# zovoilis-lab/Flye

Measured on AMD Instinct MI355X. Metric: Gbp reads overlapped/sec, higher is better.
Workload: dtype u64

## Files before the change

flye_amd/csrc/fg_ctx.h:

```cpp
#pragma once

#include <hip/hip_runtime.h>
#include <cstdint>
#include <cstdio>
#include <cstdlib>
#include <new>
#include <cstring>
#include <string>
#include <vector>
#include <map>
#include <memory>
#include <condition_variable>
#include <functional>
#include <mutex>
#include <thread>
#include <atomic>
#include <algorithm>

#include "../../include/flye_gpu.h"
#include "fg_error.h"

typedef uint64_t u64;
typedef uint32_t u32;
typedef uint16_t u16;
// ... 252 lines not shown
	std::vector<i32> hQLen;
	DevBuf<u64> dQWords, dQWordOff;
	DevBuf<i32> dQLen;

	bool indexBuilt = false;
	float sampleRate = 1.0f;
	u64 nKeys = 0, nEntries = 0, nRep = 0, tableSlots = 0;
	DevBuf<u64> dKeys;
	DevBuf<u64> dKeyOff;
	DevBuf<u64> dEntries;
	DevBuf<u64> dRepKeys;
	DevBuf<u64> dTable;
	bool tableWide = false;
	FgTable table{};
	DevBuf<u32> dIndexedBits;
	DevBuf<u32> dMaybeBits;
	u32 shardWorld = 1, shardRank = 0;

	std::unique_ptr<fg_ctx> lane2;
	std::shared_ptr<void> indexBuild;
	bool gathering = false;
	DevBuf<u64> gKeys, gKeyOff, gEntries, gRepKeys;
	u64 gNKeys = 0, gNEntries = 0, gNRep = 0;
	u32 splitWorld = 0;
	DevBuf<u64> sCounts, sEntries;
	bool scattering = false;
	u32 scatterWorld = 1, scatterRank = 0;

	DevBuf<u32> dQuery;
	u64 hitCapHint = 0;
	const u32* curQuery = nullptr;
	DevBuf<u64> dQKmerOff;
	DevBuf<u64> dProbe;
	DevBuf<u64> dPartK0, dPartV0, dPartK1, dPartV1;
	DevBuf<char> dPartScratch;
	DevBuf<unsigned long long> dPartCount;
	DevBuf<u64> dHitOff;
	DevBuf<u64> dFiltOff;
	DevBuf<i32> dFiltPos;
	DevBuf<u64> dHitKey;
	DevBuf<u32> dHitVal;
	DevBuf<u16> dHitVal16;
	bool hitVal16 = false;
	DevBuf<u32> dHitKey32;
	DevBuf<i32> dScore, dBack;
	DevBuf<int4> dCand;
	DevBuf<u64> dGroupStart;
	DevBuf<u32> dGroupQuery;
	DevBuf<u32> dGroupExt, dGroupFirstCur, dGroupLastCur;
	DevBuf<uint8_t> dGroupExtSorted;
	DevBuf<u32> dTmp32;
	DevBuf<fg_seed_hit> dSeedHits;
	DevBuf<u64> dRecvRun, dRecvIdx;
	DevBuf<u32> dRecvErr;
	DevBuf<u64> dCntA, dCntB, dGroupCnt, dGroupOff, dPrimCnt, dPrimOff, dDpGroups, dDpElems;
	DevBuf<u32> dPrimFlag, dDpSize, dListSmall, dListBig, dListDp, dListFused, dListCnt;
	DevBuf<u32> dTileCnt, dPrimPos, dScanScratch;
	DevBuf<u32> dCur, dExt;
	DevBuf<char> dPrimOut;
	DevBuf<u64> dPrimNode, dPrimBase, dMatchSize, dMatchOff, dMatches;
	DevBuf<u32> dMatchCnt;
	PinnedBuf<u64> hMatches, hMatchOff;
	PinnedBuf<u32> hMatchCnt;
	DevBuf<char> dSortTasks, dSortBig;
	DevBuf<unsigned long long> dSmallElems;
	DevBuf<unsigned long long> dLazyCnt;
// ... 385 lines not shown
```

flye_amd/csrc/fg_overlap.hip:

```cpp
#include "fg_ctx.h"
#include "fg_wavesort.h"
#include "fg_devprim.h"
#include "fg_taskchain.h"
#include <atomic>

#include <algorithm>
#include <cmath>
#include <chrono>
#include <functional>
#include <thread>
#include <type_traits>

#define WG 256
#define FLAG_SELF (1ULL << 63)
#define FLAG_FLIP (1ULL << 62)
#define OFF_MASK ((1ULL << 38) - 1)

namespace {

__device__ __forceinline__ u32 block_exscan(u32 v, u32* sh , u32* total)
{
	const int lane = threadIdx.x & 63, w = threadIdx.x >> 6;
	u32 inc = v;
	for (int o = 1; o < 64; o <<= 1)
// ... 281 lines not shown
				const u64 own = ((u64)(rec ^ (fl ? 1u : 0u)) << 32) | (u32)(fl ? L - pq - k : pq);
				if (pe >= own) pe = e;
				if (e >= own) e = entries[(so & OFF_MASK) + j + 1];
			}
			if (tieFree)
			{
				const u32 below = (u32)__builtin_amdgcn_update_dpp((int)(u32)(pe >> 32), (int)(u32)(e >> 32), 0x138, 0xf, 0xf, false);
				tied |= j > 0 && below == (u32)(e >> 32);
			}
			u32 srec = (u32)(e >> 32);
			i32 spos = (i32)(u32)e;
			if (so & FLAG_FLIP) { spos = len[srec >> 1] - spos - k; srec ^= 1u; }
			if constexpr (std::is_same<KT, fg_seed_hit>::value)
				hitKey[hbase + o] = fg_seed_hit{p0 + (i32)t, spos, firstId + srec};
			else if constexpr (std::is_same<KT, PK>::value)
				hitKey[hbase + o] = PK(((u64)srec << (curBits + FG_PK_VALBITS)) | ((u64)(u32)(p0 + (i32)t) << FG_PK_VALBITS) |
									   (u64)(u32)spos);
			else
			{
				if (sizeof(KT) == 8) hitKey[hbase + o] = (KT)(((u64)(firstId + srec) << 32) | (u32)(p0 + (i32)t));
				else hitKey[hbase + o] = (KT)((srec << curBits) | (u32)(p0 + (i32)t));
				hitVal[hbase + o] = (VT)(u32)spos;
			}
		}
		__syncthreads();
		hbase += tot;
		fbase += ftot;
	}
	if (tieFree)
	{
		const int anyTied = __syncthreads_or(tied);
		if (threadIdx.x == 0) tieFree[q] = anyTied ? 0u : 1u;
	}
}


__global__ void k_filt_pos(const u64* __restrict__ qKmerOff, const u64* __restrict__ probe, const u64* __restrict__ filtOff,
						   i32* __restrict__ filtPos)
{
	__shared__ u32 sh[WG / 64 + 1];
	const u32 q = blockIdx.x;
	const u64 a = qKmerOff[q];
	const i32 nk = (i32)(qKmerOff[q + 1] - a);
	u64 fbase = filtOff[q];
	for (i32 p0 = 0; p0 < nk; p0 += WG)
	{
		const i32 p = p0 + (i32)threadIdx.x;
		const u64 v = p < nk ? probe[a + p] : 0;
		const u32 rep = (v != 0 && (u32)(v & FG_CNT_MASK) == FG_CNT_REPETITIVE) ? 1u : 0u;
		u32 tot;
		const u32 off = block_exscan(rep, sh, &tot);
		if (rep) filtPos[fbase + off] = p;
		fbase += tot;
	}
}

__global__ void k_recv_keys(const u32* __restrict__ query, const u64* __restrict__ qKmerOff, const u64* __restrict__ qWords,
							const u64* __restrict__ qWordOff, const i32* __restrict__ qLen, const i32* __restrict__ len, int k,
							u32 firstId, u32 nRec, const fg_seed_hit* __restrict__ hits, const u64* __restrict__ run, u32 nSrc,
							const u64* __restrict__ hitOff, int recBits, int posBits, int mode, u64* __restrict__ keys,
							u64* __restrict__ vals, u64* __restrict__ hitIdx, u32* __restrict__ err)
{
	const u32 q = blockIdx.x;
	const u32 rec = query[q];
	const i32 nk = qLen[rec >> 1] - k;
	const bool rc = rec & 1;
// ... 1311 lines not shown
		const u64 n = localOff[q1] - localOff[q0];
		if (n)
		{
			c->dPartK0.reserve(n); c->dPartV0.reserve(n); c->dPartK1.reserve(n); c->dPartV1.reserve(n);
			c->dPartScratch.reserve(fgprim::radixSortScratchBytes(n));
			c->dPartCount.reserve(1);
			HIP_CHECK(hipMemsetAsync(c->dPartCount.p, 0, 8, s));
			{ ScopedK t(c->timer, "k_probe_emit");
			  hipLaunchKernelGGL(k_probe_emit, q1 - q0, WG, 0, s, q0, c->dQuery.p, qWords, qWordOff, qLen, c->dKmerOff.p, c->dQKmerOff.p,
								 c->k, c->table, regionShift, c->hasQ ? (const u32*)nullptr : c->dIndexedBits.p, probeSkipBits(c),
								 n, c->dPartK0.p, c->dPartV0.p, c->dPartCount.p); }
			unsigned long long nEmit = 0;
			HIP_CHECK(hipMemcpyAsync(&nEmit, c->dPartCount.p, 8, hipMemcpyDeviceToHost, s));
			HIP_CHECK(hipStreamSynchronize(s));
			if (nEmit > n) throw FgError{FG_ERR_HIP, "internal: more probe pairs than query k-mers"};
			if (nEmit == 0) { q0 = q1; continue; }
			int which;
			{ ScopedK t(c->timer, "k_probe_partition");
			  which = fgprim::radixSortPairs(s, c->dPartK0.p, c->dPartV0.p, c->dPartK1.p, c->dPartV1.p, nEmit, PART_KEY_BITS,
											 PART_KEY_BITS + PROBE_REGION_BITS, c->dPartScratch.p); }
			{ ScopedK t(c->timer, "k_probe");
			  hipLaunchKernelGGL(k_probe_sorted, (unsigned)((nEmit + WG - 1) / WG), WG, 0, s, which ? c->dPartK1.p : c->dPartK0.p,
								 which ? c->dPartV1.p : c->dPartV0.p, (u64)nEmit, c->table, c->dProbe.p,
								 getenv("FG_ABLATE_PROBE") ? atoi(getenv("FG_ABLATE_PROBE")) : 0); }
		}
		q0 = q1;
	}
	{ ScopedK t(c->timer, "k_probe_count");
	  hipLaunchKernelGGL(k_probe_count, nq, WG, 0, s, c->dQKmerOff.p, c->dProbe.p, c->dCntA.p, c->dCntB.p); }
}

struct ChunkResult { u64 nPrim, nHits, dpGroups, dpElems, dpElemsSmall, nMatchSlots; };

static void probeChunk(fg_ctx* c, const u32* hq, const u64* hQKmerOff, u32 qa, u32 qb, std::vector<u64>& hitsPerQuery)
{
	hipStream_t s = c->stream;
	const int k = c->k;
	const u32 nq = qb - qa;
	const u64 totalQK = hQKmerOff[qb] - hQKmerOff[qa];
	std::vector<u64> localOff(nq + 1);
	for (u32 i = 0; i <= nq; ++i) localOff[i] = hQKmerOff[qa + i] - hQKmerOff[qa];
	c->dQuery.reserve(nq); c->dQKmerOff.reserve(nq + 1);
	c->dProbe.reserve(totalQK);
	c->dHitOff.reserve(nq + 1); c->dFiltOff.reserve(nq + 1);
	c->dCntA.reserve(nq + 1); c->dCntB.reserve(nq + 1); c->dGroupCnt.reserve(nq + 1); c->dGroupOff.reserve(nq + 1);
	c->dPrimCnt.reserve(nq + 1); c->dPrimOff.reserve(nq + 1); c->dDpGroups.reserve(nq + 1); c->dDpElems.reserve(nq + 1);
	c->dListCnt.reserve(4);
	HIP_CHECK(hipMemcpyAsync(c->dQuery.p, hq + qa, nq * 4ULL, hipMemcpyHostToDevice, s));
	HIP_CHECK(hipMemcpyAsync(c->dQKmerOff.p, localOff.data(), (nq + 1) * 8ULL, hipMemcpyHostToDevice, s));

	const u64* qWords = c->hasQ ? c->dQWords.p : c->dWords.p;
	const u64* qWordOff = c->hasQ ? c->dQWordOff.p : c->dWordOff.p;
	const i32* qLen = c->hasQ ? c->dQLen.p : c->dLen.p;
	const bool partition = !c->tableWide && c->k <= 17 &&
		(getenv("FG_PROBE_PARTITION") ? atoi(getenv("FG_PROBE_PARTITION")) != 0 : false);
	if (partition) probePartitioned(c, nq, localOff.data(), qWords, qWordOff, qLen);
	else
	{ ScopedK t(c->timer, "k_probe");
	  const u32* skipBits = probeSkipBits(c);
	  if (c->tableWide)
		hipLaunchKernelGGL(k_probe<true>, nq, WG, 0, s, c->dQuery.p, qWords, qWordOff, qLen, c->dKmerOff.p,
						   c->dQKmerOff.p, k, c->table, c->hasQ ? (const u32*)nullptr : c->dIndexedBits.p, skipBits,
						   c->dProbe.p, c->dCntA.p, c->dCntB.p);
	  else
		hipLaunchKernelGGL(k_probe<false>, nq, WG, 0, s, c->dQuery.p, qWords, qWordOff, qLen, c->dKmerOff.p,
						   c->dQKmerOff.p, k, c->table, c->hasQ ? (const u32*)nullptr : c->dIndexedBits.p, skipBits,
						   c->dProbe.p, c->dCntA.p, c->dCntB.p); }
	hitsPerQuery.resize(nq);
	HIP_CHECK(hipMemcpyAsync(hitsPerQuery.data(), c->dCntA.p, nq * 8ULL, hipMemcpyDeviceToHost, s));
	HIP_CHECK(hipStreamSynchronize(s));
}

template <class KT>
static void recvFill(fg_ctx* c, const RecvHits* recv, u32 callQ0, u32 sub0, u32 nq, u64 nHits, int curBits, KT* hitKey, u32* hitVal)
{
	hipStream_t s = c->stream;
	const int k = c->k;
	const u32* dQuery = c->dQuery.p + sub0;
	const u64* dQKmerOff = c->dQKmerOff.p + sub0;
	{ ScopedK t(c->timer, "k_filt_pos");
	  hipLaunchKernelGGL(k_filt_pos, nq, WG, 0, s, dQKmerOff, c->dProbe.p, c->dFiltOff.p, c->dFiltPos.p); }
	if (nHits == 0) return;
	if (nHits > fgprim::RS_MAX_N) throw FgError{FG_ERR_ARG, "more than 2^30 - 1 seed hits in one sub-range"};
	const u32 ns = recv->nSrc;
	std::vector<u64> run(2 * (size_t)nq * ns);
	for (u32 i = 0; i < nq; ++i)
		for (u32 src = 0; src < ns; ++src)
		{
			const size_t at = (size_t)(callQ0 + sub0 + i) * ns + src;
// ... 24 lines not shown
						 c->dHitOff.p, recBits, posBits, onePass ? 0 : 1, c->dPartK0.p, c->dPartV0.p, c->dRecvIdx.p, c->dRecvErr.p); }
	if (fetchScalar(c, c->dRecvErr.p)) throw FgError{FG_ERR_ARG, "a received seed hit lies outside its query or its target"};
	u64 *k0 = c->dPartK0.p, *v0 = c->dPartV0.p, *k1 = c->dPartK1.p, *v1 = c->dPartV1.p;
	{ ScopedK t(c->timer, "k_recv_sort");
	  if (fgprim::radixSortPairs(s, k0, v0, k1, v1, nHits, 0, onePass ? gBits + storedBits : storedBits, c->dPartScratch.p))
		  { std::swap(k0, k1); std::swap(v0, v1); } }
	if (!onePass)
	{
		{ ScopedK t(c->timer, "k_recv_keys");
		  hipLaunchKernelGGL(k_recv_gkey, (unsigned)((nHits + WG - 1) / WG), WG, 0, s, v0, nHits, c->dHitOff.p, nq, dQKmerOff,
							 recv->hits, c->dRecvIdx.p, k0); }
		ScopedK t(c->timer, "k_recv_sort");
		if (fgprim::radixSortPairs(s, k0, v0, k1, v1, nHits, 0, gBits, c->dPartScratch.p)) { std::swap(k0, k1); std::swap(v0, v1); }
	}
	{ ScopedK t(c->timer, "k_recv_place");
	  hipLaunchKernelGGL(k_recv_place<KT>, (unsigned)((nHits + WG - 1) / WG), WG, 0, s, v0, nHits, recv->hits, c->dRecvIdx.p,
						 c->firstId, curBits, hitKey, hitVal); }
}

static void deviceSub(fg_ctx* c, const fg_detector_params* p, uint8_t forceLocal, u32 sub0, u32 nq, u64 primBase,
					  u64 hitCapHint , ChunkResult* res,
					  const RecvHits* recv = nullptr, u32 callQ0 = 0)
{
	hipStream_t s = c->stream;
	const int k = c->k;
	const u32* dQuery = c->dQuery.p + sub0;
	const u64* dQKmerOff = c->dQKmerOff.p + sub0;
	c->curQuery = dQuery;
	const i32* qLen = c->hasQ ? c->dQLen.p : c->dLen.p;
	c->dHitOff.reserve(nq + 1); c->dFiltOff.reserve(nq + 1);
	c->dGroupCnt.reserve(nq + 1); c->dGroupOff.reserve(nq + 1);
	c->dPrimCnt.reserve(nq + 1); c->dPrimOff.reserve(nq + 1); c->dDpGroups.reserve(nq + 1); c->dDpElems.reserve(nq + 1);
	c->dListCnt.reserve(4);
	{ ScopedK t(c->timer, "k_exscan");
	  hipLaunchKernelGGL(k_exscan, 1, 1024, 0, s, c->dCntA.p + sub0, c->dHitOff.p, nq);
	  hipLaunchKernelGGL(k_exscan, 1, 1024, 0, s, c->dCntB.p + sub0, c->dFiltOff.p, nq); }
	c->hScalar.reserve(8);
	HIP_CHECK(hipMemcpyAsync(c->hScalar.p, c->dHitOff.p + nq, 8, hipMemcpyDeviceToHost, s));
	HIP_CHECK(hipMemcpyAsync(c->hScalar.p + 1, c->dFiltOff.p + nq, 8, hipMemcpyDeviceToHost, s));
	HIP_CHECK(hipStreamSynchronize(s));
	const u64 nHits = c->hScalar.p[0], nFilt = c->hScalar.p[1];
	res->nHits = nHits;
	const u64 hitCap = std::max(nHits, hitCapHint);
	c->hitCapHint = hitCap;
	c->dFiltPos.reserve(nFilt + 1);
	int curBits = 1, recBits = 1;
	while ((1LL << curBits) < (long long)(c->hasQ ? c->qMaxLen : c->maxLen)) ++curBits;
	while ((1ULL << recBits) < 2ULL * c->nReads) ++recBits;
	const bool key32 = curBits + recBits <= 32 && !getenv("FG_FORCE_KEY64");
	c->tieFreeN = 0; c->sortReasonN = 0;
	const bool canPack = recBits + curBits + FG_PK_VALBITS <= 64 && c->maxLen < (1 << FG_PK_VALBITS);
	const bool wantPack = !(getenv("FG_PACKED_KEYS") && atoi(getenv("FG_PACKED_KEYS")) == 0);
	const int keyMode = key32 ? 0 : ((canPack && wantPack) ? 1 : 2);
	const bool val16 = keyMode == 0 && !recv && c->maxLen <= 65536 && !(getenv("FG_VAL16") && atoi(getenv("FG_VAL16")) == 0);
	c->hitVal16 = val16;
	if (keyMode == 0)
	{
		c->dHitKey32.reserve(hitCap + 1); c->dTieFree.reserve(nq + 1);
		if (val16) c->dHitVal16.reserve(hitCap + 2); else c->dHitVal.reserve(hitCap + 1);
		if (recv) recvFill<u32>(c, recv, callQ0, sub0, nq, nHits, curBits, c->dHitKey32.p, c->dHitVal.p);
		else { ScopedK t(c->timer, "k_fill");
		  if (val16)
			  hipLaunchKernelGGL((k_fill<u32, u16>), nq, WG, 0, s, dQuery, c->dLen.p, qLen, dQKmerOff, k, c->firstId, curBits,
								 c->dProbe.p, c->dEntries.p, c->dHitOff.p, c->dFiltOff.p, c->dHitKey32.p, c->dHitVal16.p, c->dFiltPos.p, c->dTieFree.p);
		  else
			  hipLaunchKernelGGL(k_fill<u32>, nq, WG, 0, s, dQuery, c->dLen.p, qLen, dQKmerOff, k, c->firstId, curBits,
								 c->dProbe.p, c->dEntries.p, c->dHitOff.p, c->dFiltOff.p, c->dHitKey32.p, c->dHitVal.p, c->dFiltPos.p, c->dTieFree.p); }
		if (!recv) { c->tieFreeQ0 = callQ0 + sub0; c->tieFreeN = nq; }
		const u32* sortFree = recv ? nullptr : c->dTieFree.p;
		if (sortFree && nHits)
		{
			c->dSortFree.reserve(nq + 1); c->dSortReason.reserve(nq + 1);
			if (sortScreen(c, c->dHitOff.p, nq, c->dHitKey32.p, curBits, recBits, c->dTieFree.p, fgChainMinUnique(p), p->min_overlap,
						   c->dSortFree.p, c->dSortReason.p))
				{ sortFree = c->dSortFree.p; c->sortReasonN = nq; }
		}
		if (val16) sortSegments<u32, u16>(c, c->dHitOff.p, nq, c->dHitKey32.p, c->dHitVal16.p, nHits, curBits, sortFree, recBits);
		else sortSegments<u32>(c, c->dHitOff.p, nq, c->dHitKey32.p, c->dHitVal.p, nHits, curBits, sortFree, recBits);
	}
	else if (keyMode == 1)
	{
		c->dHitKey.reserve(hitCap + 1);
		if (recv) recvFill<PK>(c, recv, callQ0, sub0, nq, nHits, curBits, (PK*)c->dHitKey.p, (u32*)nullptr);
		else { ScopedK t(c->timer, "k_fill");
		  hipLaunchKernelGGL(k_fill<PK>, nq, WG, 0, s, dQuery, c->dLen.p, qLen, dQKmerOff, k, c->firstId, curBits,
							 c->dProbe.p, c->dEntries.p, c->dHitOff.p, c->dFiltOff.p, (PK*)c->dHitKey.p, (u32*)nullptr, c->dFiltPos.p, (u32*)nullptr); }
		sortSegments<PK>(c, c->dHitOff.p, nq, (PK*)c->dHitKey.p, (u32*)nullptr, nHits, curBits);
	}
	else
	{
		c->dHitKey.reserve(hitCap + 1); c->dHitVal.reserve(hitCap + 1);
		if (recv) recvFill<u64>(c, recv, callQ0, sub0, nq, nHits, curBits, c->dHitKey.p, c->dHitVal.p);
		else { ScopedK t(c->timer, "k_fill");
		  hipLaunchKernelGGL(k_fill<u64>, nq, WG, 0, s, dQuery, c->dLen.p, qLen, dQKmerOff, k, c->firstId, 0,
							 c->dProbe.p, c->dEntries.p, c->dHitOff.p, c->dFiltOff.p, c->dHitKey.p, c->dHitVal.p, c->dFiltPos.p, (u32*)nullptr); }
		sortSegments<u64>(c, c->dHitOff.p, nq, c->dHitKey.p, c->dHitVal.p, nHits, curBits);
	}
	const HitKeyView<u32> hk32{c->dHitKey32.p, c->dHitVal.p, curBits, c->firstId};
	const HitKeyView<u64> hk64{c->dHitKey.p, c->dHitVal.p, curBits, c->firstId};
	const HitKeyView<PK> hkp{(const PK*)c->dHitKey.p, nullptr, curBits, c->firstId};
	const bool flat = nHits < 0xFFFFFFFFULL && !(getenv("FG_GROUP_FLAT") && atoi(getenv("FG_GROUP_FLAT")) == 0);
	const u64 nTiles = (nHits + FG_GROUP_TILE - 1) / FG_GROUP_TILE;
	u64 nGroups = 0;
	if (!flat)
	{
		{ ScopedK t(c->timer, "k_group_count");
		  if (keyMode == 0) hipLaunchKernelGGL(k_group_count<u32>, nq, WG, 0, s, c->dHitOff.p, hk32, c->dGroupCnt.p);
		  else if (keyMode == 1) hipLaunchKernelGGL(k_group_count<PK>, nq, WG, 0, s, c->dHitOff.p, hkp, c->dGroupCnt.p);
		  else hipLaunchKernelGGL(k_group_count<u64>, nq, WG, 0, s, c->dHitOff.p, hk64, c->dGroupCnt.p); }
		{ ScopedK t(c->timer, "k_exscan");
		  hipLaunchKernelGGL(k_exscan, 1, 1024, 0, s, c->dGroupCnt.p, c->dGroupOff.p, nq); }
		nGroups = fetchScalar(c, c->dGroupOff.p + nq);
	}
	else if (nTiles)
	{
		c->dTileCnt.reserve(nTiles + 1); c->dScanScratch.reserve(fgprim::scanScratchElems(nTiles + 1));
		{ ScopedK t(c->timer, "k_group_count");
		  if (keyMode == 0) hipLaunchKernelGGL((k_group_count_flat<u32, FG_GROUP_GF>), (unsigned)nTiles, WG, 0, s, c->dHitOff.p, nq, hk32, nHits, c->dTileCnt.p);
		  else if (keyMode == 1) hipLaunchKernelGGL((k_group_count_flat<PK, FG_GROUP_GF>), (unsigned)nTiles, WG, 0, s, c->dHitOff.p, nq, hkp, nHits, c->dTileCnt.p);
		  else hipLaunchKernelGGL((k_group_count_flat<u64, FG_GROUP_GF>), (unsigned)nTiles, WG, 0, s, c->dHitOff.p, nq, hk64, nHits, c->dTileCnt.p); }
		{ ScopedK t(c->timer, "k_group_scan");
		  fgprim::scan<u32>(s, c->dTileCnt.p, c->dTileCnt.p, nTiles + 1, false, c->dScanScratch.p); }
		nGroups = fetchScalar(c, c->dTileCnt.p + nTiles);
	}
	if (nGroups >= 0xFFFFFFFFULL) throw FgError{FG_ERR_ARG, "too many target groups in one chunk"};
// ... 106 lines not shown
	  }
	  HIP_CHECK(hipMemcpyAsync(c->hOff.p + 3 * (size_t)(nq + 1), c->dSmallElems.p, 24, hipMemcpyDeviceToHost, s));
	  HIP_CHECK(hipEventRecord(c->evOff, s));
	  static const int wantPieces = getenv("FG_D2H_PIECES") ? std::max(1, std::min(FG_D2H_MAX_PIECES, atoi(getenv("FG_D2H_PIECES")))) : 12;
	  const int nPieces = nPrim >= 100000 ? wantPieces : 1;
	  for (int i = 0; i < nPieces; ++i)
	  {
		  const u64 a = nPrim * i / nPieces, b = nPrim * (i + 1) / nPieces;
		  if (b > a)
			  HIP_CHECK(hipMemcpyAsync(c->hPrim.p + (primBase + a) * sizeof(PrimRec), c->dPrimOut.p + a * sizeof(PrimRec),
									   (b - a) * sizeof(PrimRec), hipMemcpyDeviceToHost, s));
		  HIP_CHECK(hipEventRecord(c->evPiece[i], s));
		  c->pieceEnd[i] = primBase + b;
	  }
	  c->nPieces = nPieces; }
	HIP_CHECK(hipEventSynchronize(c->evOff));
	if (keepAln) HIP_CHECK(hipStreamSynchronize(s));
	res->nPrim = nPrim;
	res->dpGroups = 0; res->dpElems = 0;
	res->dpElemsSmall = c->hOff.p[3 * (size_t)(nq + 1)];
	if (flat) { res->dpGroups = c->hOff.p[3 * (size_t)(nq + 1) + 1]; res->dpElems = c->hOff.p[3 * (size_t)(nq + 1) + 2]; }
	else for (u32 i = 0; i < nq; ++i) { res->dpGroups += c->hOff.p[(nq + 1) + i]; res->dpElems += c->hOff.p[2 * (size_t)(nq + 1) + i]; }
}

static void stageBudgets(fg_ctx* c, u64& kmerBudget, u64& hitBudget)
{
	kmerBudget = getenv("FG_KMER_BUDGET") ? strtoull(getenv("FG_KMER_BUDGET"), nullptr, 10) : (1ULL << 30);
	hitBudget = getenv("FG_HIT_BUDGET") ? strtoull(getenv("FG_HIT_BUDGET"), nullptr, 10) : (3ULL << 29);
	if (!getenv("FG_KMER_BUDGET") && !getenv("FG_HIT_BUDGET"))
	{
		size_t freeB = 0, totalB = 0;
		HIP_CHECK(hipMemGetInfo(&freeB, &totalB));
		const u64 held = c->dHitKey.bytes() + c->dHitKey32.bytes() + c->dHitVal.bytes() + c->dHitVal16.bytes() + c->dCur.bytes() + c->dExt.bytes() +
						 c->dScore.bytes() + c->dBack.bytes() + c->dTmp32.bytes() + c->dCand.bytes() + c->dProbe.bytes();
		const u64 avail = (u64)freeB + held;
		const u64 usable = avail > (8ULL << 30) ? (avail - (4ULL << 30)) / 10 * 9 : avail / 2;
		hitBudget = std::min(hitBudget, std::max<u64>(16ULL << 20, usable / 100 * 85 / 80));
		kmerBudget = std::min(kmerBudget, std::max<u64>(16ULL << 20, usable / 100 * 15 / 9));
	}
}

static fg_ctx* laneTwo(fg_ctx* c)
{
	if (!c->lane2)
	{
		std::unique_ptr<fg_ctx> l(new fg_ctx);
		l->device = c->device;
		if (hipStreamCreateWithFlags(&l->stream, hipStreamNonBlocking) != hipSuccess ||
			hipStreamCreateWithFlags(&l->stream2, hipStreamNonBlocking) != hipSuccess ||
			hipStreamCreateWithFlags(&l->stream3, hipStreamNonBlocking) != hipSuccess ||
			hipEventCreateWithFlags(&l->evJoin3, hipEventDisableTiming) != hipSuccess ||
			hipEventCreateWithFlags(&l->evOff, hipEventDisableTiming) != hipSuccess ||
			hipEventCreateWithFlags(&l->evFork, hipEventDisableTiming) != hipSuccess ||
			hipEventCreateWithFlags(&l->evJoin, hipEventDisableTiming) != hipSuccess)
			throw FgError{FG_ERR_HIP, "streams of the second lane"};
		for (auto& e : l->evPiece)
			if (hipEventCreateWithFlags(&e, hipEventDisableTiming) != hipSuccess) throw FgError{FG_ERR_HIP, "events of the second lane"};
		l->timer.stream = l->stream;
		c->lane2 = std::move(l);
	}
	fg_ctx* l = c->lane2.get();
	l->k = c->k; l->nReads = c->nReads; l->firstId = c->firstId; l->maxLen = c->maxLen;
	l->totalKmers = c->totalKmers; l->totalBases = c->totalBases;
	l->hasQ = c->hasQ; l->nQReads = c->nQReads; l->qFirstId = c->qFirstId; l->qMaxLen = c->qMaxLen;
	l->indexBuilt = c->indexBuilt; l->sampleRate = c->sampleRate; l->nKeys = c->nKeys; l->nEntries = c->nEntries; l->nRep = c->nRep;
	l->tableSlots = c->tableSlots; l->tableWide = c->tableWide; l->table = c->table;
	l->timer.enabled = c->timer.enabled;
	l->dWords.alias(c->dWords); l->dWordOff.alias(c->dWordOff); l->dLen.alias(c->dLen); l->dKmerOff.alias(c->dKmerOff);
	l->dQWords.alias(c->dQWords); l->dQWordOff.alias(c->dQWordOff); l->dQLen.alias(c->dQLen);
	l->dKeyOff.alias(c->dKeyOff); l->dEntries.alias(c->dEntries); l->dTable.alias(c->dTable); l->dIndexedBits.alias(c->dIndexedBits); l->dMaybeBits.alias(c->dMaybeBits);
	l->dQuery.alias(c->dQuery); l->dQKmerOff.alias(c->dQKmerOff); l->dProbe.alias(c->dProbe);
	l->dCntA.alias(c->dCntA); l->dCntB.alias(c->dCntB);
	l->dLazyCnt.alias(c->dLazyCnt);
	return l;
}

struct SubResult {
	u32 qa = 0, qb = 0;
	int lane = 0;
	u64 lanePrimBase = 0;
	ChunkResult cr{};
	std::vector<u64> primOff;
	std::vector<u64> mData, mOff;
};

void fgOverlaps(fg_ctx* c, const fg_detector_params* p, const u32* queryIds, u32 nq, i32 maxOverlaps,
				uint8_t forceLocal, fg_overlap_batch* out, const RecvHits* recv)
{
	hipStream_t s = c->stream;
	const int k = c->k;
	c->timer.reset();
	c->hitCapHint = 0;
	const auto tHost0 = std::chrono::steady_clock::now();
	struct EvPair {
		KernelTimer& t; hipEvent_t a, b;
		explicit EvPair(KernelTimer& t_) : t(t_), a(t_.get()), b(nullptr) { try { b = t_.get(); } catch (...) { t_.pool.push_back(a); throw; } }
		~EvPair() { t.pool.push_back(a); t.pool.push_back(b); }
	} evp(c->timer);
	const hipEvent_t evA = evp.a, evB = evp.b;
	HIP_CHECK(hipEventRecord(evA, s));
	c->dLazyCnt.reserve(FG_LAZY_STRIPES * 8);
	HIP_CHECK(hipMemsetAsync(c->dLazyCnt.p, 0, FG_LAZY_STRIPES * 8 * sizeof(unsigned long long), s));

	BatchOwner* own = BatchOwner::acquire();
	out->owner_ = own;
	out->n_queries = nq;
	own->queryOff.assign(nq + 1, 0);
	own->statOff.assign(nq + 1, 0);

	std::vector<u32> hq(nq);
	std::vector<u64> hQKmerOff(nq + 1, 0);
	u64 queryBp = 0;
	const int STAT_WND = 10000;
	u64 statCap = 0;
	for (u32 i = 0; i < nq; ++i)
	{
		hq[i] = queryIds[i] - (c->hasQ ? c->qFirstId : c->firstId);
		const i32 L = (c->hasQ ? c->hQLen : c->hLen)[hq[i] >> 1];
		hQKmerOff[i + 1] = hQKmerOff[i] + (u64)std::max(0, L - k);
		queryBp += L;
		statCap += (u64)(L / STAT_WND + 1);
	}
	out->query_bp = queryBp;
	out->query_kmers = hQKmerOff[nq];
	if (nq == 0)
	{
		out->query_off = own->queryOff.data(); out->div_stats_off = own->statOff.data();
		if (p->keep_alignment) { own->matchOff.assign(1, 0); out->match_off = own->matchOff.data(); }
		if (p->partition_bad_mappings) { own->needsTrim.assign(1, 0); out->needs_trim = own->needsTrim.data(); }
		return;
	}
#ifdef FG_SORT_ABLATE
	if (getenv("FG_ABLATE"))
	{
		const int ab = atoi(getenv("FG_ABLATE"));
		HIP_CHECK(hipMemcpyToSymbol(HIP_SYMBOL(wsort::g_ablate), &ab, sizeof(int)));
	}
#endif

	u64 kmerBudget, hitBudget;
	stageBudgets(c, kmerBudget, hitBudget);
	if (recv) hitBudget = std::min<u64>(hitBudget * 2 / 3, 1ULL << 29);
	std::vector<std::pair<u32, u32>> chunks;
	{
		u32 qa = 0;
		while (qa < nq)
		{
			u32 qb = qa + 1;
			while (qb < nq && hQKmerOff[qb + 1] - hQKmerOff[qa] <= kmerBudget) ++qb;
			chunks.push_back({qa, qb});
			qa = qb;
		}
	}
	const bool keepAln = p->keep_alignment;
	std::vector<u64> mData, mOff(1, 0);
	std::vector<u64> primOffAll(nq + 1, 0);
	std::vector<const PrimRec*> primPtr(nq, nullptr);
	std::vector<u64> hitsPerQuery;
	u64 nPrim = 0;
	out->seed_hits = 0; out->dp_groups = 0; out->dp_elements = 0; out->dp_elements_small = 0;
	const int nLanes = getenv("FG_LANES") ? std::max(1, std::min(2, atoi(getenv("FG_LANES")))) : 2;
	const u64 laneMinHits = getenv("FG_LANE_MIN_HITS") ? strtoull(getenv("FG_LANE_MIN_HITS"), nullptr, 10) : (48ULL << 20);
	const u32 laneSplit = getenv("FG_LANE_SPLIT") ? (u32)std::max(2, atoi(getenv("FG_LANE_SPLIT"))) : 4u;
	bool laned = false;
	u64 lanePrim[2] = {0, 0};
	std::vector<std::unique_ptr<SubResult>> subs;
	for (const auto& ch : chunks)
	{
		probeChunk(c, hq.data(), hQKmerOff.data(), ch.first, ch.second, hitsPerQuery);
		const u32 cn = ch.second - ch.first;
		if (recv)
		{
			hitsPerQuery.assign(recv->total + ch.first, recv->total + ch.second);
			HIP_CHECK(hipMemcpyAsync(c->dCntA.p, hitsPerQuery.data(), cn * 8ULL, hipMemcpyHostToDevice, s));
			HIP_CHECK(hipStreamSynchronize(s));
		}
		u64 chunkHits = 0;
		for (u32 i = 0; i < cn; ++i) chunkHits += hitsPerQuery[i];
		const bool forcedCut = getenv("FG_LANE_MIN_HITS") && chunkHits >= laneMinHits && cn >= 2 * laneSplit;
		const bool twoLanes = nLanes == 2 && (chunkHits > hitBudget || forcedCut);
		const u64 budget = !twoLanes ? hitBudget
			: (chunkHits > hitBudget ? std::max<u64>(1, hitBudget / 2) : std::max<u64>(1, (chunkHits + laneSplit - 1) / laneSplit));
		std::vector<std::pair<u32, u32>> ranges;
		u64 maxSubHits = 0;
		std::vector<u64> cuts;
		if (twoLanes && getenv("FG_LANE_FRACS") && chunkHits / 2 <= hitBudget)
		{
			u64 accPct = 0;
			for (const char* q = getenv("FG_LANE_FRACS"); *q;)
			{
				accPct += strtoull(q, (char**)&q, 10);
				if (*q == ',') ++q;
				cuts.push_back(chunkHits / 100 * std::min<u64>(accPct, 100));
			}
		}
		size_t cutI = 0;
		u64 before = 0;
		for (u32 sa = 0; sa < cn;)
		{
			u32 sb = sa + 1;
			u64 acc = hitsPerQuery[sa];
			if (!cuts.empty())
// ... 348 lines not shown
```

Before: 5.543.

## Probe and fill seeds in fixed-size k-mer tiles instead of per-query blocks

Adds tile-based probe and fill kernels. Each workgroup handles a fixed 1024-kmer tile of a query rather than a whole query. The probe compacts non-zero results with their positions and records per-tile hit and filter counts. Those counts are scanned to produce hit offsets, and the fill kernel expands hits per tile using shared-memory owner search. The aim is to fix load imbalance from long and variable-length reads and to raise parallelism. The cost is extra buffers (probe positions as u16, tile arrays), more kernel launches and scans, and a smaller k-mer budget to make room for the position array.

```diff
diff --git a/flye_amd/csrc/fg_ctx.h b/flye_amd/csrc/fg_ctx.h
--- a/flye_amd/csrc/fg_ctx.h
+++ b/flye_amd/csrc/fg_ctx.h
@@ -308,6 +308,13 @@
 	const u32* curQuery = nullptr;
 	DevBuf<u64> dQKmerOff;
 	DevBuf<u64> dProbe;
+	bool seedTiles = false;
+	DevBuf<u16> dProbePos;
+	std::vector<u32> hTileOff;
+	DevBuf<u32> dTileOff, dTileN, dTileFilt;
+	DevBuf<u64> dTileHits;
+	DevBuf<u64> dTileHitBase, dTileScan64;
+	DevBuf<u32> dTileFiltBase, dTileScan32;
 	DevBuf<u64> dPartK0, dPartV0, dPartK1, dPartV1;
 	DevBuf<char> dPartScratch;
 	DevBuf<unsigned long long> dPartCount;
diff --git a/flye_amd/csrc/fg_overlap.hip b/flye_amd/csrc/fg_overlap.hip
--- a/flye_amd/csrc/fg_overlap.hip
+++ b/flye_amd/csrc/fg_overlap.hip
@@ -337,6 +337,392 @@
 		const int anyTied = __syncthreads_or(tied);
 		if (threadIdx.x == 0) tieFree[q] = anyTied ? 0u : 1u;
 	}
+}
+
+#define SEED_TILE (WG * 4)
+
+__device__ __forceinline__ u32 tile_query(const u32* __restrict__ tileOff, u32 nq, u32 t)
+{
+	u32 lo = 0, hi = nq;
+	while (hi - lo > 1)
+	{
+		const u32 m = lo + ((hi - lo) >> 1);
+		if (fg_uni(tileOff[m]) <= t) lo = m; else hi = m;
+	}
+	return lo;
+}
+
+template <bool WIDE>
+__global__ void __launch_bounds__(WG) k_probe_tile(const u32* __restrict__ query, const u64* __restrict__ words,
+		const u64* __restrict__ wordOff, const i32* __restrict__ len, const u64* __restrict__ kmerOff,
+		const u64* __restrict__ qKmerOff, const u32* __restrict__ tileOff, u32 nq, int k, FgTable table,
+		const u32* __restrict__ indexedBits, const u32* __restrict__ maybeBits, u64* __restrict__ probe,
+		u16* __restrict__ probePos, u32* __restrict__ tileN, u64* __restrict__ tileHits, u32* __restrict__ tileFilt)
+{
+	constexpr int FI = SEED_TILE / WG;
+	__shared__ u32 sh[WG / 64 + 1];
+	__shared__ u64 shH[WG / 64];
+	__shared__ u32 shF[WG / 64];
+	const u32 t = blockIdx.x;
+	const u32 q = tile_query(tileOff, nq, t);
+	const i32 p0 = (i32)((t - fg_uni(tileOff[q])) * (u32)SEED_TILE);
+	const u32 rec = query[q];
+	const u32 r = rec >> 1;
+	const bool rc = rec & 1;
+	const i32 nk = len[r] - k;
+	const u64* w = words + wordOff[r];
+	const u64 kbase = (indexedBits || maybeBits) ? kmerOff[r] : 0;
+	const u64 tbase = qKmerOff[q] + (u64)p0;
+	const i32 lastWord = (len[r] - 1) >> 5;
+	i32 qf[FI];
+	u32 selfBit[FI];
+	bool act[FI];
+	{
+		u32 selfWord[FI], maybeWord[FI];
+		u64 bit[FI];
+		bool in[FI], has[FI];
+#pragma unroll
+		for (int i = 0; i < FI; ++i)
+		{
+			const i32 p = p0 + (i32)threadIdx.x * FI + i;
+			in[i] = p < nk;
+			const i32 pc = in[i] ? p : nk - 1;
+			qf[i] = rc ? nk - pc : pc;
+			has[i] = qf[i] < nk;
+			bit[i] = kbase + (u64)(has[i] ? qf[i] : 0);
+			selfWord[i] = 0u; maybeWord[i] = ~0u;
+		}
+		if (indexedBits)
+		{
+#pragma unroll
+			for (int i = 0; i < FI; ++i) selfWord[i] = indexedBits[bit[i] >> 5];
+		}
+		if (maybeBits)
+		{
+#pragma unroll
+			for (int i = 0; i < FI; ++i) maybeWord[i] = maybeBits[bit[i] >> 5];
+		}
+#pragma unroll
+		for (int i = 0; i < FI; ++i)
+		{
+			selfBit[i] = (in[i] && has[i]) ? ((selfWord[i] >> (bit[i] & 31)) & 1u) : 0u;
+			act[i] = in[i] && (!has[i] || ((maybeWord[i] >> (bit[i] & 31)) & 1u));
+		}
+	}
+	u64 key[FI];
+	bool flip[FI], pal[FI];
+	{
+		u64 w0[FI], w1[FI];
+#pragma unroll
+		for (int i = 0; i < FI; ++i)
+		{
+			const i32 i0 = qf[i] >> 5;
+			w0[i] = w[i0];
+			w1[i] = w[i0 < lastWord ? i0 + 1 : lastWord];
+		}
+		const u64 mask = (k == 32) ? ~0ULL : ((1ULL << (2 * k)) - 1);
+#pragma unroll
+		for (int i = 0; i < FI; ++i)
+		{
+			const int shf = (qf[i] & 31) * 2;
+			u64 x = w0[i] >> shf;
+			if (shf + 2 * k > 64) x |= w1[i] << ((64 - shf) & 63);
+			x &= mask;
+			const u64 a = fg_rev2(x, k), b = ~x & mask;
+			const u64 fw = rc ? b : a, rv = rc ? a : b;
+			flip[i] = rv < fw;
+			pal[i] = fw == rv;
+			key[i] = flip[i] ? rv : fw;
+		}
+	}
+	u64 v[FI];
+	if constexpr (WIDE)
+	{
+#pragma unroll
+		for (int i = 0; i < FI; ++i) v[i] = act[i] ? fg_probe<true>(table, key[i]) : 0ULL;
+	}
+	else
+	{
+		const bool onePart = table.nParts <= 1;
+		u32 part[FI], grp[FI];
+		u64 slot[FI], kb[FI];
+		if (onePart)
+		{
+#pragma unroll
+			for (int i = 0; i < FI; ++i)
+			{
+				part[i] = 0;
+				grp[i] = __umulhi((u32)(fg_mix(key[i]) >> 32), table.groups[0]);
+				slot[i] = table.slotBase[0] + (act[i] ? (u64)grp[i] * 8u : 0ULL);
+				kb[i] = table.keyBase[0];
+			}
+		}
+		else
+		{
+#pragma unroll
+			for (int i = 0; i < FI; ++i)
+			{
+				u32 pt = 0;
+				while (pt + 1 < table.nParts && key[i] >= table.bound[pt + 1]) ++pt;
+				part[i] = pt;
+				grp[i] = __umulhi((u32)(fg_mix(key[i]) >> 32), table.groups[pt]);
+				slot[i] = act[i] ? table.slotBase[pt] + (u64)grp[i] * 8u : table.slotBase[0];
+				kb[i] = table.keyBase[pt];
+			}
+		}
+		ulonglong2 ln[FI][4];
+#pragma unroll
+		for (int i = 0; i < FI; ++i)
+		{
+			const ulonglong2* g = (const ulonglong2*)(table.slots + slot[i]);
+			ln[i][0] = g[0]; ln[i][1] = g[1]; ln[i][2] = g[2]; ln[i][3] = g[3];
+		}
+		u64 hit[FI];
+		bool spill = false;
+#pragma unroll
+		for (int i = 0; i < FI; ++i)
+		{
+			const u64 sl[8] = {ln[i][0].x, ln[i][0].y, ln[i][1].x, ln[i][1].y, ln[i][2].x, ln[i][2].y, ln[i][3].x, ln[i][3].y};
+			u64 h = FG_EMPTY_KEY;
+			bool empty = false;
+#pragma unroll
+			for (int j = 0; j < 8; ++j)
+			{
+				if ((sl[j] >> FG_IDX_BITS) == key[i]) h = sl[j];
+				empty |= sl[j] == FG_EMPTY_KEY;
+			}
+			hit[i] = act[i] ? h : FG_EMPTY_KEY;
+			act[i] = act[i] && h == FG_EMPTY_KEY && !empty;
+			spill |= act[i];
+		}
+		if (spill)
+		{
+#pragma unroll
+			for (int i = 0; i < FI; ++i)
+				if (act[i]) hit[i] = fg_probe_slot(table, part[i], grp[i] + 1 == table.groups[part[i]] ? 0 : grp[i] + 1, key[i]);
+		}
+		u64 idx[FI];
+		bool bounds[FI];
+		bool any = false;
+#pragma unroll
+		for (int i = 0; i < FI; ++i)
+		{
+			const bool found = hit[i] != FG_EMPTY_KEY;
+			const bool rep = found && (hit[i] & FG_IDX_MASK) == FG_IDX_MASK;
+			bounds[i] = found && !rep;
+			idx[i] = bounds[i] ? kb[i] + (hit[i] & FG_IDX_MASK) : 0ULL;
+			v[i] = rep ? (u64)FG_CNT_REPETITIVE : 0ULL;
+			any |= bounds[i];
+		}
+		if (__ballot(any) != 0)
+		{
+			u64 lo[FI], hi[FI];
+#pragma unroll
+			for (int i = 0; i < FI; ++i) { lo[i] = table.keyOff[idx[i]]; hi[i] = table.keyOff[idx[i] + (bounds[i] ? 1 : 0)]; }
+#pragma unroll
+			for (int i = 0; i < FI; ++i) if (bounds[i]) v[i] = (lo[i] << FG_CNT_BITS) | (hi[i] - lo[i]);
+		}
+	}
+	u64 hits = 0;
+	u32 filt = 0, nz = 0;
+#pragma unroll
+	for (int i = 0; i < FI; ++i)
+	{
+		if (v[i] == 0) continue;
+		++nz;
+		const u32 cnt = (u32)(v[i] & FG_CNT_MASK);
+		if (cnt == FG_CNT_REPETITIVE) ++filt;
+		else
+		{
+			const u32 self = selfBit[i] && !(rc && pal[i]);
+			hits += cnt - self;
+			if (self) v[i] |= FLAG_SELF;
+			if (flip[i]) v[i] |= FLAG_FLIP;
+		}
+	}
+	u32 n;
+	u32 rank = block_exscan(nz, sh, &n);
+#pragma unroll
+	for (int i = 0; i < FI; ++i)
+		if (v[i] != 0)
+		{
+			probe[tbase + rank] = v[i];
+			probePos[tbase + rank] = (u16)(threadIdx.x * FI + i);
+			++rank;
+		}
+	for (int o = 32; o > 0; o >>= 1) { hits += __shfl_down(hits, o); filt += __shfl_down(filt, o); }
+	if ((threadIdx.x & 63) == 0) { shH[threadIdx.x >> 6] = hits; shF[threadIdx.x >> 6] = filt; }
+	__syncthreads();
+	if (threadIdx.x == 0)
+	{
+		u64 h = 0; u32 f = 0;
+		for (int i = 0; i < WG / 64; ++i) { h += shH[i]; f += shF[i]; }
+		tileN[t] = n; tileHits[t] = h; tileFilt[t] = f;
+	}
+}
+
+__global__ void k_tile_totals(const u32* __restrict__ tileOff, u32 nq, const u64* __restrict__ tileHits,
+							  const u32* __restrict__ tileFilt, u64* __restrict__ hitCnt, u64* __restrict__ filtCnt)
+{
+	const u32 q = blockIdx.x * WG + threadIdx.x;
+	if (q >= nq) return;
+	u64 h = 0, f = 0;
+	for (u32 t = tileOff[q]; t < tileOff[q + 1]; ++t) { h += tileHits[t]; f += tileFilt[t]; }
+	hitCnt[q] = h; filtCnt[q] = f;
+}
+
+__global__ void k_tile_offsets(const u32* __restrict__ tileOff, u32 nq, const u64* __restrict__ hitBase,
+							   const u32* __restrict__ filtBase, u64* __restrict__ hitOff, u64* __restrict__ filtOff)
+{
+	const u32 q = blockIdx.x * WG + threadIdx.x;
+	if (q > nq) return;
+	const u32 t = tileOff[q] - tileOff[0];
+	hitOff[q] = hitBase[t]; filtOff[q] = filtBase[t];
+}
+
+template <class KT, class VT = u32>
+__global__ void __launch_bounds__(WG) k_fill_tile(const u32* __restrict__ query, const i32* __restrict__ len,
+		const i32* __restrict__ qLen, const u64* __restrict__ qKmerOff, const u32* __restrict__ tileOff, u32 nq, int k,
+		u32 firstId, int curBits, const u64* __restrict__ probe, const u16* __restrict__ probePos,
+		const u32* __restrict__ tileN, const u64* __restrict__ entries, const u64* __restrict__ tileHitBase,
+		const u32* __restrict__ tileFiltBase, KT* __restrict__ hitKey, VT* __restrict__ hitVal, i32* __restrict__ filtPos,
+		u32* __restrict__ tieFree)
+{
+	constexpr int FI = SEED_TILE / WG;
+	static_assert((SEED_TILE & (SEED_TILE - 1)) == 0, "the owner search halves the tile exactly");
+	__shared__ u32 sh[WG / 64 + 1];
+	__shared__ u32 sStart[SEED_TILE + 1];
+	__shared__ u64 sOff[SEED_TILE];
+	__shared__ u16 sPos[SEED_TILE];
+	__shared__ u32 sRec[3][FI][WG / 64];
+	const u32 t = fg_uni(tileOff[0]) + blockIdx.x;
+	const u32 n = fg_uni(tileN[t]);
+	if (n == 0) return;
+	const u32 q = tile_query(tileOff, nq, t);
+	const i32 p0 = (i32)((t - fg_uni(tileOff[q])) * (u32)SEED_TILE);
+	const u32 rec = query[q];
+	const i32 L = qLen[rec >> 1];
+	const u64 tbase = qKmerOff[q] + (u64)p0;
+	const u64 hbase = tileHitBase[blockIdx.x];
+	const u64 fbase = tileFiltBase[blockIdx.x];
+	{
+		u64 vv[FI];
+		u32 eff[FI], pp[FI];
+		u32 effSum = 0, repSum = 0;
+#pragma unroll
+		for (int i = 0; i < FI; ++i)
+		{
+			const u32 e = threadIdx.x * FI + i;
+			const u64 v = e < n ? probe[tbase + e] : 0;
+			pp[i] = e < n ? probePos[tbase + e] : 0;
+			u32 cnt = (u32)(v & FG_CNT_MASK);
+			const bool rep = (cnt == FG_CNT_REPETITIVE);
+			if (rep) cnt = 0;
+			const bool hasSelf = cnt && (v & FLAG_SELF);
+			eff[i] = cnt - (hasSelf ? 1u : 0u);
+			vv[i] = (((v >> FG_CNT_BITS) & OFF_MASK) | (v & FLAG_FLIP) | (hasSelf ? FLAG_SELF : 0ULL));
+			if (rep) { vv[i] = ~0ULL; ++repSum; }
+			effSum += eff[i];
+		}
+		u32 tot0, ftot;
+		u32 start = block_exscan(effSum, sh, &tot0);
+		u32 fstart = block_exscan(repSum, sh, &ftot);
+#pragma unroll
+		for (int i = 0; i < FI; ++i)
+		{
+			const u32 e = threadIdx.x * FI + i;
+			const bool rep = vv[i] == ~0ULL;
+			if (rep) filtPos[fbase + fstart++] = p0 + (i32)pp[i];
+			sStart[e] = start;
+			sOff[e] = rep ? 0ULL : vv[i];
+			sPos[e] = (u16)pp[i];
+			start += eff[i];
+		}
+		if (threadIdx.x == 0) sStart[SEED_TILE] = tot0;
+	}
+	__syncthreads();
+	const u32 tot = sStart[SEED_TILE];
+	bool tied = false;
+	u32 turn = 0;
+	for (u32 o0 = 0; o0 < tot; o0 += SEED_TILE, ++turn)
+	{
+		bool ok[FI];
+		u32 own[FI], jj[FI];
+		u64 so[FI], e[FI];
+#pragma unroll
+		for (int i = 0; i < FI; ++i)
+		{
+			const u32 o = o0 + (u32)i * WG + threadIdx.x;
+			ok[i] = o < tot;
+			u32 lo = 0;
+#pragma unroll
+			for (u32 half = SEED_TILE >> 1; half; half >>= 1) if (sStart[lo + half] <= o) lo += half;
+			own[i] = lo;
+			jj[i] = o - sStart[lo];
+			so[i] = sOff[lo];
+		}
+		u64 eb[FI], at[FI];
+		bool self[FI];
+#pragma unroll
+		for (int i = 0; i < FI; ++i)
+		{
+			self[i] = ok[i] && (so[i] & FLAG_SELF);
+			at[i] = ok[i] ? (so[i] & OFF_MASK) + jj[i] : 0ULL;
+		}
+#pragma unroll
+		for (int i = 0; i < FI; ++i) { e[i] = entries[at[i]]; eb[i] = entries[at[i] + (self[i] ? 1 : 0)]; }
+#pragma unroll
+		for (int i = 0; i < FI; ++i)
+		{
+			if (self[i])
+			{
+				const i32 pq = p0 + (i32)sPos[own[i]];
+				const bool fl = so[i] & FLAG_FLIP;
+				const u64 ownE = ((u64)(rec ^ (fl ? 1u : 0u)) << 32) | (u32)(fl ? L - pq - k : pq);
+				if (e[i] >= ownE) e[i] = eb[i];
+			}
+		}
+		if (tieFree)
+		{
+			const u32 w = threadIdx.x >> 6;
+			if ((threadIdx.x & 63) == 63)
+			{
+#pragma unroll
+				for (int i = 0; i < FI; ++i) sRec[turn % 3][i][w] = (u32)(e[i] >> 32);
+			}
+			__syncthreads();
+#pragma unroll
+			for (int i = 0; i < FI; ++i)
+			{
+				const u32 edge = w > 0 ? sRec[turn % 3][i][w - 1]
+									   : (i > 0 ? sRec[turn % 3][i > 0 ? i - 1 : 0][WG / 64 - 1] : sRec[(turn + 2) % 3][FI - 1][WG / 64 - 1]);
+				const u32 below = (u32)__builtin_amdgcn_update_dpp((int)edge, (int)(u32)(e[i] >> 32), 0x138, 0xf, 0xf, false);
+				tied |= ok[i] && jj[i] > 0 && below == (u32)(e[i] >> 32);
+			}
+		}
+		i32 tl[FI];
+#pragma unroll
+		for (int i = 0; i < FI; ++i) tl[i] = len[(ok[i] && (so[i] & FLAG_FLIP)) ? (u32)(e[i] >> 32) >> 1 : 0u];
+#pragma unroll
+		for (int i = 0; i < FI; ++i)
+		{
+			if (!ok[i]) continue;
+			const u64 o = hbase + o0 + (u32)i * WG + threadIdx.x;
+			const u32 cur = (u32)(p0 + (i32)sPos[own[i]]);
+			u32 srec = (u32)(e[i] >> 32);
+			i32 spos = (i32)(u32)e[i];
+			if (so[i] & FLAG_FLIP) { spos = tl[i] - spos - k; srec ^= 1u; }
+			if constexpr (std::is_same<KT, PK>::value)
+				hitKey[o] = PK(((u64)srec << (curBits + FG_PK_VALBITS)) | ((u64)cur << FG_PK_VALBITS) | (u64)(u32)spos);
+			else
+			{
+				if (sizeof(KT) == 8) hitKey[o] = (KT)(((u64)(firstId + srec) << 32) | cur);
+				else hitKey[o] = (KT)((srec << curBits) | cur);
+				hitVal[o] = (VT)(u32)spos;
+			}
+		}
+	}
+	if (tieFree && __ballot(tied) != 0 && (threadIdx.x & 63) == 0) tieFree[q] = 0u;
 }
 
 
@@ -1714,7 +2100,8 @@
 
 struct ChunkResult { u64 nPrim, nHits, dpGroups, dpElems, dpElemsSmall, nMatchSlots; };
 
-static void probeChunk(fg_ctx* c, const u32* hq, const u64* hQKmerOff, u32 qa, u32 qb, std::vector<u64>& hitsPerQuery)
+static void probeChunk(fg_ctx* c, const u32* hq, const u64* hQKmerOff, u32 qa, u32 qb, std::vector<u64>& hitsPerQuery,
+					   const u32* hTileOff = nullptr)
 {
 	hipStream_t s = c->stream;
 	const int k = c->k;
@@ -1736,7 +2123,34 @@
 	const i32* qLen = c->hasQ ? c->dQLen.p : c->dLen.p;
 	const bool partition = !c->tableWide && c->k <= 17 &&
 		(getenv("FG_PROBE_PARTITION") ? atoi(getenv("FG_PROBE_PARTITION")) != 0 : false);
+	const bool tiles = hTileOff && !partition && !(getenv("FG_SEED_TILES") && atoi(getenv("FG_SEED_TILES")) == 0);
+	c->seedTiles = tiles;
 	if (partition) probePartitioned(c, nq, localOff.data(), qWords, qWordOff, qLen);
+	else if (tiles)
+	{
+		c->hTileOff.resize(nq + 1);
+		for (u32 i = 0; i <= nq; ++i) c->hTileOff[i] = hTileOff[qa + i] - hTileOff[qa];
+		const u32 nT = c->hTileOff[nq];
+		c->dTileOff.reserve(nq + 1); c->dProbePos.reserve(totalQK);
+		c->dTileN.reserve(nT + 1); c->dTileHits.reserve(nT + 1); c->dTileFilt.reserve(nT + 1);
+		HIP_CHECK(hipMemcpyAsync(c->dTileOff.p, c->hTileOff.data(), (nq + 1) * 4ULL, hipMemcpyHostToDevice, s));
+		HIP_CHECK(hipMemsetAsync(c->dTileHits.p + nT, 0, 8, s));
+		HIP_CHECK(hipMemsetAsync(c->dTileFilt.p + nT, 0, 4, s));
+		const u32* skipBits = probeSkipBits(c);
+		const u32* selfBits = c->hasQ ? (const u32*)nullptr : c->dIndexedBits.p;
+		{ ScopedK t(c->timer, "k_probe");
+		if (nT && c->tableWide)
+			hipLaunchKernelGGL(k_probe_tile<true>, nT, WG, 0, s, c->dQuery.p, qWords, qWordOff, qLen, c->dKmerOff.p, c->dQKmerOff.p,
+							   c->dTileOff.p, nq, k, c->table, selfBits, skipBits, c->dProbe.p, c->dProbePos.p, c->dTileN.p,
+							   c->dTileHits.p, c->dTileFilt.p);
+		else if (nT)
+			hipLaunchKernelGGL(k_probe_tile<false>, nT, WG, 0, s, c->dQuery.p, qWords, qWordOff, qLen, c->dKmerOff.p, c->dQKmerOff.p,
+							   c->dTileOff.p, nq, k, c->table, selfBits, skipBits, c->dProbe.p, c->dProbePos.p, c->dTileN.p,
+							   c->dTileHits.p, c->dTileFilt.p); }
+		ScopedK t(c->timer, "k_tile_totals");
+		hipLaunchKernelGGL(k_tile_totals, (nq + WG - 1) / WG, WG, 0, s, c->dTileOff.p, nq, c->dTileHits.p, c->dTileFilt.p,
+						   c->dCntA.p, c->dCntB.p);
+	}
 	else
 	{ ScopedK t(c->timer, "k_probe");
 	  const u32* skipBits = probeSkipBits(c);
@@ -1827,9 +2241,34 @@
 	c->dGroupCnt.reserve(nq + 1); c->dGroupOff.reserve(nq + 1);
 	c->dPrimCnt.reserve(nq + 1); c->dPrimOff.reserve(nq + 1); c->dDpGroups.reserve(nq + 1); c->dDpElems.reserve(nq + 1);
 	c->dListCnt.reserve(4);
+	const bool tiles = c->seedTiles && !recv;
+	const u32* dTileOff = tiles ? c->dTileOff.p + sub0 : nullptr;
+	const u32 tile0 = tiles ? c->hTileOff[sub0] : 0, nSeedTiles = tiles ? c->hTileOff[sub0 + nq] - tile0 : 0;
+	if (tiles)
+	{
+		c->dTileHitBase.reserve(nSeedTiles + 1); c->dTileFiltBase.reserve(nSeedTiles + 1);
+		c->dTileScan64.reserve(fgprim::scanScratchElems(nSeedTiles + 1)); c->dTileScan32.reserve(fgprim::scanScratchElems(nSeedTiles + 1));
+		ScopedK t(c->timer, "k_exscan");
+		fgprim::scan<u64>(s, c->dTileHits.p + tile0, c->dTileHitBase.p, nSeedTiles + 1, false, c->dTileScan64.p);
+		fgprim::scan<u32>(s, c->dTileFilt.p + tile0, c->dTileFiltBase.p, nSeedTiles + 1, false, c->dTileScan32.p);
+		hipLaunchKernelGGL(k_tile_offsets, (nq + 1 + WG - 1) / WG, WG, 0, s, dTileOff, nq, c->dTileHitBase.p, c->dTileFiltBase.p,
+						   c->dHitOff.p, c->dFiltOff.p);
+	}
+	else
 	{ ScopedK t(c->timer, "k_exscan");
 	  hipLaunchKernelGGL(k_exscan, 1, 1024, 0, s, c->dCntA.p + sub0, c->dHitOff.p, nq);
 	  hipLaunchKernelGGL(k_exscan, 1, 1024, 0, s, c->dCntB.p + sub0, c->dFiltOff.p, nq); }
+	auto fillTiles = [&](auto* hitKey, auto* hitVal, int cb, u32* tie)
+	{
+		using KT = std::remove_pointer_t<decltype(hitKey)>;
+		using VT = std::remove_pointer_t<decltype(hitVal)>;
+		ScopedK t(c->timer, "k_fill");
+		if (tie) HIP_CHECK(hipMemsetD32Async((hipDeviceptr_t)tie, 1, nq, s));
+		if (!nSeedTiles) return;
+		hipLaunchKernelGGL((k_fill_tile<KT, VT>), nSeedTiles, WG, 0, s, dQuery, c->dLen.p, qLen, dQKmerOff, dTileOff, nq, k, c->firstId, cb,
+						   c->dProbe.p, c->dProbePos.p, c->dTileN.p, c->dEntries.p, c->dTileHitBase.p, c->dTileFiltBase.p,
+						   hitKey, hitVal, c->dFiltPos.p, tie);
+	};
 	c->hScalar.reserve(8);
 	HIP_CHECK(hipMemcpyAsync(c->hScalar.p, c->dHitOff.p + nq, 8, hipMemcpyDeviceToHost, s));
 	HIP_CHECK(hipMemcpyAsync(c->hScalar.p + 1, c->dFiltOff.p + nq, 8, hipMemcpyDeviceToHost, s));
@@ -1854,6 +2293,11 @@
 		c->dHitKey32.reserve(hitCap + 1); c->dTieFree.reserve(nq + 1);
 		if (val16) c->dHitVal16.reserve(hitCap + 2); else c->dHitVal.reserve(hitCap + 1);
 		if (recv) recvFill<u32>(c, recv, callQ0, sub0, nq, nHits, curBits, c->dHitKey32.p, c->dHitVal.p);
+		else if (tiles)
+		{
+			if (val16) fillTiles(c->dHitKey32.p, c->dHitVal16.p, curBits, c->dTieFree.p);
+			else fillTiles(c->dHitKey32.p, c->dHitVal.p, curBits, c->dTieFree.p);
+		}
 		else { ScopedK t(c->timer, "k_fill");
 		  if (val16)
 			  hipLaunchKernelGGL((k_fill<u32, u16>), nq, WG, 0, s, dQuery, c->dLen.p, qLen, dQKmerOff, k, c->firstId, curBits,
@@ -1877,6 +2321,7 @@
 	{
 		c->dHitKey.reserve(hitCap + 1);
 		if (recv) recvFill<PK>(c, recv, callQ0, sub0, nq, nHits, curBits, (PK*)c->dHitKey.p, (u32*)nullptr);
+		else if (tiles) fillTiles((PK*)c->dHitKey.p, (u32*)nullptr, curBits, (u32*)nullptr);
 		else { ScopedK t(c->timer, "k_fill");
 		  hipLaunchKernelGGL(k_fill<PK>, nq, WG, 0, s, dQuery, c->dLen.p, qLen, dQKmerOff, k, c->firstId, curBits,
 							 c->dProbe.p, c->dEntries.p, c->dHitOff.p, c->dFiltOff.p, (PK*)c->dHitKey.p, (u32*)nullptr, c->dFiltPos.p, (u32*)nullptr); }
@@ -1886,6 +2331,7 @@
 	{
 		c->dHitKey.reserve(hitCap + 1); c->dHitVal.reserve(hitCap + 1);
 		if (recv) recvFill<u64>(c, recv, callQ0, sub0, nq, nHits, curBits, c->dHitKey.p, c->dHitVal.p);
+		else if (tiles) fillTiles(c->dHitKey.p, c->dHitVal.p, 0, (u32*)nullptr);
 		else { ScopedK t(c->timer, "k_fill");
 		  hipLaunchKernelGGL(k_fill<u64>, nq, WG, 0, s, dQuery, c->dLen.p, qLen, dQKmerOff, k, c->firstId, 0,
 							 c->dProbe.p, c->dEntries.p, c->dHitOff.p, c->dFiltOff.p, c->dHitKey.p, c->dHitVal.p, c->dFiltPos.p, (u32*)nullptr); }
@@ -2058,11 +2504,11 @@
 		size_t freeB = 0, totalB = 0;
 		HIP_CHECK(hipMemGetInfo(&freeB, &totalB));
 		const u64 held = c->dHitKey.bytes() + c->dHitKey32.bytes() + c->dHitVal.bytes() + c->dHitVal16.bytes() + c->dCur.bytes() + c->dExt.bytes() +
-						 c->dScore.bytes() + c->dBack.bytes() + c->dTmp32.bytes() + c->dCand.bytes() + c->dProbe.bytes();
+						 c->dScore.bytes() + c->dBack.bytes() + c->dTmp32.bytes() + c->dCand.bytes() + c->dProbe.bytes() + c->dProbePos.bytes();
 		const u64 avail = (u64)freeB + held;
 		const u64 usable = avail > (8ULL << 30) ? (avail - (4ULL << 30)) / 10 * 9 : avail / 2;
 		hitBudget = std::min(hitBudget, std::max<u64>(16ULL << 20, usable / 100 * 85 / 80));
-		kmerBudget = std::min(kmerBudget, std::max<u64>(16ULL << 20, usable / 100 * 15 / 9));
+		kmerBudget = std::min(kmerBudget, std::max<u64>(16ULL << 20, usable / 100 * 15 / 11));
 	}
 }
 
@@ -2096,6 +2542,9 @@
 	l->dQWords.alias(c->dQWords); l->dQWordOff.alias(c->dQWordOff); l->dQLen.alias(c->dQLen);
 	l->dKeyOff.alias(c->dKeyOff); l->dEntries.alias(c->dEntries); l->dTable.alias(c->dTable); l->dIndexedBits.alias(c->dIndexedBits); l->dMaybeBits.alias(c->dMaybeBits);
 	l->dQuery.alias(c->dQuery); l->dQKmerOff.alias(c->dQKmerOff); l->dProbe.alias(c->dProbe);
+	l->seedTiles = c->seedTiles; l->hTileOff = c->hTileOff;
+	l->dProbePos.alias(c->dProbePos); l->dTileOff.alias(c->dTileOff); l->dTileN.alias(c->dTileN); l->dTileHits.alias(c->dTileHits);
+	l->dTileFilt.alias(c->dTileFilt);
 	l->dCntA.alias(c->dCntA); l->dCntB.alias(c->dCntB);
 	l->dLazyCnt.alias(c->dLazyCnt);
 	return l;
@@ -2136,6 +2585,7 @@
 
 	std::vector<u32> hq(nq);
 	std::vector<u64> hQKmerOff(nq + 1, 0);
+	std::vector<u32> hTileOff(nq + 1, 0);
 	u64 queryBp = 0;
 	const int STAT_WND = 10000;
 	u64 statCap = 0;
@@ -2144,6 +2594,7 @@
 		hq[i] = queryIds[i] - (c->hasQ ? c->qFirstId : c->firstId);
 		const i32 L = (c->hasQ ? c->hQLen : c->hLen)[hq[i] >> 1];
 		hQKmerOff[i + 1] = hQKmerOff[i] + (u64)std::max(0, L - k);
+		hTileOff[i + 1] = hTileOff[i] + (u32)((std::max(0, L - k) + SEED_TILE - 1) / SEED_TILE);
 		queryBp += L;
 		statCap += (u64)(L / STAT_WND + 1);
 	}
@@ -2193,7 +2644,7 @@
 	std::vector<std::unique_ptr<SubResult>> subs;
 	for (const auto& ch : chunks)
 	{
-		probeChunk(c, hq.data(), hQKmerOff.data(), ch.first, ch.second, hitsPerQuery);
+		probeChunk(c, hq.data(), hQKmerOff.data(), ch.first, ch.second, hitsPerQuery, recv ? nullptr : hTileOff.data());
 		const u32 cn = ch.second - ch.first;
 		if (recv)
 		{
```

Result: faster. 5.614, median of 6 (+1.3%).
